# ggerganov/ggml

Measured on NVIDIA H100. Metric: mul_mat_q4_K_4096x11008_n1_weight_throughput, higher is better.
Workload: dtype int8 x int4 (q4_K weights x q8_K activations, dp4a), f32 accumulate

## Files before the change

### ggml_b200/csrc/b200_mm_plan.h

```cpp
#pragma once

#include "b200_internal.h"
#include "b200_quants.cuh"
#include "b200_sb_tasks.cuh"
#include "b200_sb_mma.cuh"

namespace b200 {

struct tma_params {
    const uint8_t * w;
    const float *   x;
    float *         y;
    size_t          nb11;
    int64_t         M, K;
    int32_t         N;
    int32_t         row_bytes;
    int32_t         RB;
    int32_t         P, G;
    int32_t         nchunks;
    int32_t         stage_bytes;
    int32_t         nstages;
    act_layout      L;
};

struct tma_plan {
    tma_params p;
    int grid, block, smem, nc, r;
};

struct sb_params {
    const uint8_t * w; const float * x; float * y;
    int64_t M, K;
    int32_t row_bytes, rows_per_chunk, nchunks, stage_bytes, nstages, ntasks_row;
    unsigned int * counters;
    unsigned int * ctl;
    int32_t ncols; int64_t x_stride;
    int32_t src1_static;
    int32_t src0_static;
    int32_t static_chunks;
    int64_t l2_prefetch_bytes;
    const float * ep_bias; float * ep_y2; float * ep_y3; const float * ep_res;
    unsigned long long * dbg;
    int32_t world, rank;
    int64_t row_offset;
    uint32_t epoch;
    float *    y_peers[8];
    uint32_t * flag_peers[8];
    sb_act A;
};

struct sb_plan { sb_params p; int grid, smem, nw, nc; bool two; };

struct mma_params {
    const uint8_t * w; const float * x; float * y;
    int64_t M, K;
    int32_t row_bytes, ntiles, nslices, ks, ntask_row, pitch, stage_bytes, nstages;
    unsigned int * counters;
    int32_t ncols; int64_t x_stride;
    int32_t src1_static, src0_static;
    int64_t l2_prefetch_bytes;
    const uint8_t * rec_global;
    mma_act A;
};

struct mma_plan { mma_params p; int grid, smem, ng; size_t workspace; };

struct tc2_plan {
    int BN, m_tiles, n_tiles, splitk, chunks, nstages, smem, grid;
    size_t xb_bytes, partial_bytes, scale_bytes, workspace;
};

struct dense_plan { ggml_b200_mul_mat_args b; size_t wbytes; tc2_plan tc; size_t workspace; };

struct mmid_g_plan { int BN, m_tiles, max_tiles, chunks, nstages, smem; size_t xb_bytes, scale_bytes, tab_bytes, perm_bytes, workspace; int64_t n_pairs; };

enum route_kind {
    R_GENERIC,
    R_TMA,
    R_TMA_UNFIT,
    R_SB,
    R_SB_GROUPS,
    R_MMA,
    R_WGMMA,
    R_DENSE,
};

struct mm_plan {
    route_kind kind;
    int64_t group;
    size_t workspace;
    tma_plan tma;
    sb_plan sb, sb_tail;
    mma_plan mma;
    tc2_plan wgmma;
    dense_plan dense;
};

}
```

### ggml_b200/csrc/b200_sb_tasks.cuh

```cuda
#pragma once
#include "b200_quants.cuh"

namespace b200 {

#ifndef B200_HOST_EMU
__device__ __forceinline__ int dp4a_us(uint32_t a, int b, int c) {
    int d;
    asm("dp4a.u32.s32 %0, %1, %2, %3;" : "=r"(d) : "r"(a), "r"(b), "r"(c));
    return d;
}
#else
inline int dp4a_us(uint32_t a, int b, int c) { for (int i = 0; i < 4; ++i) c += (int)((a >> (8 * i)) & 0xFF) * (int)(int8_t)(b >> (8 * i)); return c; }
#endif

template <int T> struct sbfmt;
template <> struct sbfmt<T_Q4_K> { static constexpr int TASK_W = 256, TASK_B = 144, LPR = 16, KQ = 1; };
template <> struct sbfmt<T_Q5_K> { static constexpr int TASK_W = 256, TASK_B = 176, LPR = 16, KQ = 1; };
template <> struct sbfmt<T_Q6_K> { static constexpr int TASK_W = 256, TASK_B = 210, LPR = 16, KQ = 1; };
template <> struct sbfmt<T_Q4_0> { static constexpr int TASK_W = 256, TASK_B = 144, LPR = 16, KQ = 0; };
template <> struct sbfmt<T_Q8_0> { static constexpr int TASK_W = 128, TASK_B = 136, LPR = 32, KQ = 0; };
template <> struct sbfmt<T_Q5_0> { static constexpr int TASK_W = 256, TASK_B = 176, LPR = 16, KQ = 0; };
template <> struct sbfmt<T_IQ4_NL> { static constexpr int TASK_W = 256, TASK_B = 144, LPR = 16, KQ = 0; };
template <> struct sbfmt<T_IQ4_XS> { static constexpr int TASK_W = 256, TASK_B = 136, LPR = 16, KQ = 1; };
template <> struct sbfmt<T_Q4_1> { static constexpr int TASK_W = 256, TASK_B = 160, LPR = 16, KQ = 0; };
// ... 262 lines not shown
        tot -= 32 * off;
#pragma unroll
        for (int j = 0; j < 2; ++j) {
            int p[4] = { 0, 0, 0, 0 };
            const int4 yv0 = lds128(a + (8 * h + j) * 16), yv1 = lds128(a + (8 * h + j + 2) * 16);
            const int4 yv2 = lds128(a + (8 * h + j + 4) * 16), yv3 = lds128(a + (8 * h + j + 6) * 16);
            const int ya[4] = { yv0.x, yv0.y, yv0.z, yv0.w }, yb[4] = { yv1.x, yv1.y, yv1.z, yv1.w };
            const int yc[4] = { yv2.x, yv2.y, yv2.z, yv2.w }, yd4[4] = { yv3.x, yv3.y, yv3.z, yv3.w };
#pragma unroll
            for (int i = 0; i < 4; ++i) {
                const uint32_t la = word(16 * h + 4 * j + i), lb = word(16 * h + 8 + 4 * j + i), qh = word(32 + 8 * h + 4 * j + i);
                p[0] = __dp4a((int)((la & 0x0F0F0F0F)        | ((qh << 4) & 0x30303030)), ya[i], p[0]);
                p[1] = __dp4a((int)((lb & 0x0F0F0F0F)        | ((qh << 2) & 0x30303030)), yb[i], p[1]);
                p[2] = __dp4a((int)(((la >> 4) & 0x0F0F0F0F) | ( qh       & 0x30303030)), yc[i], p[2]);
                p[3] = __dp4a((int)(((lb >> 4) & 0x0F0F0F0F) | ((qh >> 2) & 0x30303030)), yd4[i], p[3]);
            }
            if (j == 0) tot += sbyte<0>(scw0) * p[0] + sbyte<2>(scw0) * p[1] + sbyte<0>(scw1) * p[2] + sbyte<2>(scw1) * p[3];
            else        tot += sbyte<1>(scw0) * p[0] + sbyte<3>(scw0) * p[1] + sbyte<1>(scw1) * p[2] + sbyte<3>(scw1) * p[3];
        }
    }
    const float d = h2f(word(52) & 0xFFFF) * *(const float *)(a + SB_OFF_D);
    return d * (float)tot;
}

template <> __device__ __forceinline__ float task_dot<T_Q5_0>(const uint8_t * w, const uint8_t * rec, int t) {
    const uint8_t * a = rec + (size_t)t * SB_REC;
    uint32_t ww[45];
#pragma unroll
    for (int i = 0; i < 11; ++i) { const int4 v = lds128(w + 16 * i); ww[4 * i] = v.x; ww[4 * i + 1] = v.y; ww[4 * i + 2] = v.z; ww[4 * i + 3] = v.w; }
    ww[44] = 0;
    const int4 sa = lds128(a + SB_OFF_S32), sb = lds128(a + SB_OFF_S32 + 16);
    const int s32[8] = { sa.x, sa.y, sa.z, sa.w, sb.x, sb.y, sb.z, sb.w };
    const int4 da = lds128(a + SB_OFF_D), db = lds128(a + SB_OFF_D + 16);
    const float yd[8] = { __int_as_float(da.x), __int_as_float(da.y), __int_as_float(da.z), __int_as_float(da.w),
                          __int_as_float(db.x), __int_as_float(db.y), __int_as_float(db.z), __int_as_float(db.w) };
    float acc = 0.0f;
#pragma unroll
    for (int b = 0; b < 8; ++b) {
        const int w0 = (22 * b) / 4;
        const bool odd = (b & 1) != 0;
        uint32_t q[4], dbits, qh;
        if (!odd) {
            dbits = ww[w0] & 0xFFFF;
            qh = __funnelshift_r(ww[w0], ww[w0 + 1], 16);
#pragma unroll
            for (int i = 0; i < 4; ++i) q[i] = __funnelshift_r(ww[w0 + 1 + i], ww[w0 + 2 + i], 16);
        } else {
            dbits = ww[w0] >> 16;
            qh = ww[w0 + 1];
#pragma unroll
            for (int i = 0; i < 4; ++i) q[i] = ww[w0 + 2 + i];
        }
        const int4 ylo = lds128(a + (2 * b) * 16), yhi = lds128(a + (2 * b + 1) * 16);
        const int y[8] = { ylo.x, ylo.y, ylo.z, ylo.w, yhi.x, yhi.y, yhi.z, yhi.w };
        const int s = q5_block_dot(q, qh, y) - 16 * s32[b];
        acc += (h2f(dbits) * yd[b]) * (float)s;
    }
    return acc;
}

template <> __device__ __forceinline__ float task_dot<T_IQ4_NL>(const uint8_t * w, const uint8_t * rec, int t) {
    const uint8_t * a = rec + (size_t)t * SB_REC;
    uint32_t ww[37];
#pragma unroll
    for (int i = 0; i < 9; ++i) { const int4 v = lds128(w + 16 * i); ww[4 * i] = v.x; ww[4 * i + 1] = v.y; ww[4 * i + 2] = v.z; ww[4 * i + 3] = v.w; }
    ww[36] = 0;
    const int4 da = lds128(a + SB_OFF_D), db = lds128(a + SB_OFF_D + 16);
    const float yd[8] = { __int_as_float(da.x), __int_as_float(da.y), __int_as_float(da.z), __int_as_float(da.w),
                          __int_as_float(db.x), __int_as_float(db.y), __int_as_float(db.z), __int_as_float(db.w) };
    float acc = 0.0f;
#pragma unroll
    for (int b = 0; b < 8; ++b) {
        const int w0 = (18 * b) / 4;
        const bool odd = (b & 1) != 0;
        uint32_t q[4], dbits;
        if (!odd) {
            dbits = ww[w0] & 0xFFFF;
#pragma unroll
            for (int i = 0; i < 4; ++i) q[i] = __funnelshift_r(ww[w0 + i], ww[w0 + i + 1], 16);
        } else {
            dbits = ww[w0] >> 16;
#pragma unroll
            for (int i = 0; i < 4; ++i) q[i] = ww[w0 + 1 + i];
        }
        const int4 ylo = lds128(a + (2 * b) * 16), yhi = lds128(a + (2 * b + 1) * 16);
        const int yl[4] = { ylo.x, ylo.y, ylo.z, ylo.w }, yh[4] = { yhi.x, yhi.y, yhi.z, yhi.w };
        int s = 0;
#pragma unroll
        for (int i = 0; i < 4; ++i) {
            s = __dp4a((int)iq4nl_lookup4(q[i]), yl[i], s);
            s = __dp4a((int)iq4nl_lookup4(q[i] >> 4), yh[i], s);
        }
        acc += (yd[b] * h2f(dbits)) * (float)s;
    }
    return acc;
}

template <> __device__ __forceinline__ float task_dot<T_IQ4_XS>(const uint8_t * w, const uint8_t * rec, int t) {
    const uint8_t * a = rec + (size_t)t * SB_REC;
    uint32_t ww[34];
#pragma unroll
    for (int i = 0; i < 17; ++i) { const uint2 v = *(const uint2 *)(w + 8 * i); ww[2 * i] = v.x; ww[2 * i + 1] = v.y; }
    int tot = 0;
#pragma unroll
    for (int ib = 0; ib < 8; ++ib) {
        const int4 ylo = lds128(a + (2 * ib) * 16), yhi = lds128(a + (2 * ib + 1) * 16);
        const int yl[4] = { ylo.x, ylo.y, ylo.z, ylo.w }, yh[4] = { yhi.x, yhi.y, yhi.z, yhi.w };
        int s = 0;
#pragma unroll
        for (int i = 0; i < 4; ++i) {
            s = __dp4a((int)iq4nl_lookup4(ww[2 + 4 * ib + i]), yl[i], s);
            s = __dp4a((int)iq4nl_lookup4(ww[2 + 4 * ib + i] >> 4), yh[i], s);
        }
        tot += iq4xs_scale(ww[0], ww[1], ib) * s;
    }
    return (h2f(ww[0] & 0xFFFF) * *(const float *)(a + SB_OFF_D)) * (float)tot;
}

__device__ __forceinline__ void sb_load_q8_1_s(const uint8_t * a, float (&ys)[8]) {
    const int4 sv = lds128(a + SB_OFF_H32);
    const uint32_t u[4] = { (uint32_t)sv.x, (uint32_t)sv.y, (uint32_t)sv.z, (uint32_t)sv.w };
#pragma unroll
    for (int i = 0; i < 4; ++i) { ys[2 * i] = h2f(u[i] & 0xFFFF); ys[2 * i + 1] = h2f(u[i] >> 16); }
}
template <> __device__ __forceinline__ float task_dot<T_Q4_1>(const uint8_t * w, const uint8_t * rec, int t) {
    const uint8_t * a = rec + (size_t)t * SB_REC;
    uint32_t ww[40];
#pragma unroll
    for (int i = 0; i < 10; ++i) { const int4 v = lds128(w + 16 * i); ww[4 * i] = v.x; ww[4 * i + 1] = v.y; ww[4 * i + 2] = v.z; ww[4 * i + 3] = v.w; }
    const int4 da = lds128(a + SB_OFF_D), db = lds128(a + SB_OFF_D + 16);
    const float yd[8] = { __int_as_float(da.x), __int_as_float(da.y), __int_as_float(da.z), __int_as_float(da.w),
                          __int_as_float(db.x), __int_as_float(db.y), __int_as_float(db.z), __int_as_float(db.w) };
    float ys[8];
    sb_load_q8_1_s(a, ys);
    float acc = 0.0f;
#pragma unroll
    for (int b = 0; b < 8; ++b) {
        const int4 ylo = lds128(a + (2 * b) * 16), yhi = lds128(a + (2 * b + 1) * 16);
        const int yl[4] = { ylo.x, ylo.y, ylo.z, ylo.w }, yh[4] = { yhi.x, yhi.y, yhi.z, yhi.w };
        int p0 = 0, p1 = 0;
#pragma unroll
        for (int i = 0; i < 4; ++i) {
            p0 = __dp4a((int)(ww[5 * b + 1 + i] & 0x0F0F0F0F), yl[i], p0);
            p1 = dp4a_us(ww[5 * b + 1 + i] & 0xF0F0F0F0u, yh[i], p1);
        }
        acc += (h2f(ww[5 * b] & 0xFFFF) * yd[b]) * (float)(p0 + (p1 >> 4)) + h2f(ww[5 * b] >> 16) * ys[b];
    }
    return acc;
}
template <> __device__ __forceinline__ float task_dot<T_Q5_1>(const uint8_t * w, const uint8_t * rec, int t) {
    const uint8_t * a = rec + (size_t)t * SB_REC;
    uint32_t ww[48];
#pragma unroll
    for (int i = 0; i < 12; ++i) { const int4 v = lds128(w + 16 * i); ww[4 * i] = v.x; ww[4 * i + 1] = v.y; ww[4 * i + 2] = v.z; ww[4 * i + 3] = v.w; }
    const int4 da = lds128(a + SB_OFF_D), db = lds128(a + SB_OFF_D + 16);
    const float yd[8] = { __int_as_float(da.x), __int_as_float(da.y), __int_as_float(da.z), __int_as_float(da.w),
                          __int_as_float(db.x), __int_as_float(db.y), __int_as_float(db.z), __int_as_float(db.w) };
    float ys[8];
    sb_load_q8_1_s(a, ys);
    float acc = 0.0f;
#pragma unroll
    for (int b = 0; b < 8; ++b) {
        const int4 ylo = lds128(a + (2 * b) * 16), yhi = lds128(a + (2 * b + 1) * 16);
        const int y[8] = { ylo.x, ylo.y, ylo.z, ylo.w, yhi.x, yhi.y, yhi.z, yhi.w };
        const uint32_t q[4] = { ww[6 * b + 2], ww[6 * b + 3], ww[6 * b + 4], ww[6 * b + 5] };
        const int s = q5_block_dot(q, ww[6 * b + 1], y);
        acc += (h2f(ww[6 * b] & 0xFFFF) * yd[b]) * (float)s + h2f(ww[6 * b] >> 16) * ys[b];
    }
    return acc;
}

template <> __device__ __forceinline__ float task_dot<T_Q2_K>(const uint8_t * w, const uint8_t * rec, int t) {
    const uint8_t * a = rec + (size_t)t * SB_REC;
    const uint32_t * wp = (const uint32_t *)w;
    const int4 sa = lds128(a + SB_OFF_S16), sb = lds128(a + SB_OFF_S16 + 16);
    const int s16w[8] = { sa.x, sa.y, sa.z, sa.w, sb.x, sb.y, sb.z, sb.w };
    int isum = 0, msum = 0;
#pragma unroll
    for (int k = 0; k < 4; ++k) {
        const uint32_t scw = wp[k];
        const uint32_t mins = (scw >> 4) & 0x0F0F0F0Fu, scs = scw & 0x0F0F0F0Fu;
        msum = dp2a_lo_su(s16w[2 * k], mins, msum);
        msum = dp2a_hi_su(s16w[2 * k + 1], mins, msum);
#pragma unroll
        for (int gg = 0; gg < 4; ++gg) {
            const int g = 4 * k + gg, h = g >> 3, jj = (g >> 1) & 3, half16 = g & 1;
            const int4 yv = lds128(a + g * 16);
            const int y[4] = { yv.x, yv.y, yv.z, yv.w };
            int p = 0;
#pragma unroll
            for (int i = 0; i < 4; ++i) p = __dp4a((int)((wp[4 + 8 * h + 4 * half16 + i] >> (2 * jj)) & 0x03030303u), y[i], p);
            const int sc = gg == 0 ? ubyte<0>(scs) : gg == 1 ? ubyte<1>(scs) : gg == 2 ? ubyte<2>(scs) : ubyte<3>(scs);
            isum += sc * p;
        }
    }
    const float yd = *(const float *)(a + SB_OFF_D);
    const float dall = yd * h2f(wp[20] & 0xFFFF), dmin = yd * h2f(wp[20] >> 16);
    return dall * (float)isum - dmin * (float)msum;
}

template <> __device__ __forceinline__ float task_dot<T_Q3_K>(const uint8_t * w, const uint8_t * rec, int t) {
    const uint8_t * a = rec + (size_t)t * SB_REC;
    const uint32_t sh = ((uint32_t)(uintptr_t)w & 2) * 8;
    const uint32_t * wa = (const uint32_t *)((uintptr_t)w & ~(uintptr_t)3);
    auto word = [&](int i) { return __funnelshift_r(wa[i], wa[i + 1], sh); };
    const uint32_t s0 = word(24), s1 = word(25), s2 = word(26);
    const uint32_t aux[4] = { ( s0       & 0x0F0F0F0Fu) | (( s2       & 0x03030303u) << 4),
                              ( s1       & 0x0F0F0F0Fu) | (((s2 >> 2) & 0x03030303u) << 4),
                              ((s0 >> 4) & 0x0F0F0F0Fu) | (((s2 >> 4) & 0x03030303u) << 4),
                              ((s1 >> 4) & 0x0F0F0F0Fu) | (((s2 >> 6) & 0x03030303u) << 4) };
    int isum = 0;
#pragma unroll
    for (int g = 0; g < 16; ++g) {
        const int h = g >> 3, jj = (g >> 1) & 3, half16 = g & 1, bit = 4 * h + jj;
        const int4 yv = lds128(a + g * 16);
        const int y[4] = { yv.x, yv.y, yv.z, yv.w };
        int p = 0, low = 0;
#pragma unroll
        for (int i = 0; i < 4; ++i) {
            p   = __dp4a((int)((word(8 + 8 * h + 4 * half16 + i) >> (2 * jj)) & 0x03030303u), y[i], p);
            low = __dp4a((int)(~(word(4 * half16 + i) >> bit) & 0x01010101u), y[i], low);
        }
        const uint32_t ax = aux[g >> 2];
        const int sc = ((g & 3) == 0 ? ubyte<0>(ax) : (g & 3) == 1 ? ubyte<1>(ax) : (g & 3) == 2 ? ubyte<2>(ax) : ubyte<3>(ax)) - 32;
        isum += sc * (p - 4 * low);
    }
    return (h2f(word(27) & 0xFFFF) * *(const float *)(a + SB_OFF_D)) * (float)isum;
}

template <int C, bool FIVE>
__device__ __forceinline__ void q45_chunk2(const uint8_t * qs0, const uint8_t * qs1, const uint32_t (&qh0)[8], const uint32_t (&qh1)[8], const uint8_t * a,
                                            int sa0, int sa1, int sb0, int sb1, int & acc0, int & acc1) {
    const int4 qa0 = lds128(qs0 + 32 * C), qb0 = lds128(qs0 + 32 * C + 16), qa1 = lds128(qs1 + 32 * C), qb1 = lds128(qs1 + 32 * C + 16);
    const uint32_t q0[8] = { (uint32_t)qa0.x, (uint32_t)qa0.y, (uint32_t)qa0.z, (uint32_t)qa0.w, (uint32_t)qb0.x, (uint32_t)qb0.y, (uint32_t)qb0.z, (uint32_t)qb0.w };
    const uint32_t q1[8] = { (uint32_t)qa1.x, (uint32_t)qa1.y, (uint32_t)qa1.z, (uint32_t)qa1.w, (uint32_t)qb1.x, (uint32_t)qb1.y, (uint32_t)qb1.z, (uint32_t)qb1.w };
    int p00 = 0, p01 = 0, p10 = 0, p11 = 0;
#pragma unroll
    for (int h = 0; h < 2; ++h) {
        const int4 ylo = lds128(a + (4 * C + h) * 16), yhi = lds128(a + (4 * C + 2 + h) * 16);
        const int yl[4] = { ylo.x, ylo.y, ylo.z, ylo.w }, yh[4] = { yhi.x, yhi.y, yhi.z, yhi.w };
#pragma unroll
        for (int i = 0; i < 4; ++i) {
            const uint32_t x0 = q0[4 * h + i], x1 = q1[4 * h + i];
            if constexpr (FIVE) {
                const uint32_t h0 = qh0[4 * h + i] >> (2 * C), h1 = qh1[4 * h + i] >> (2 * C);
                p00 = __dp4a((int)((x0 & 0x0F0F0F0F) | ((h0 & 0x01010101) << 4)), yl[i], p00);
                p01 = __dp4a((int)(((x0 >> 4) & 0x0F0F0F0F) | ((h0 & 0x02020202) << 3)), yh[i], p01);
                p10 = __dp4a((int)((x1 & 0x0F0F0F0F) | ((h1 & 0x01010101) << 4)), yl[i], p10);
                p11 = __dp4a((int)(((x1 >> 4) & 0x0F0F0F0F) | ((h1 & 0x02020202) << 3)), yh[i], p11);
            } else {
                p00 = __dp4a((int)(x0 & 0x0F0F0F0F), yl[i], p00);
                p01 = dp4a_us(x0 & 0xF0F0F0F0u, yh[i], p01);
                p10 = __dp4a((int)(x1 & 0x0F0F0F0F), yl[i], p10);
                p11 = dp4a_us(x1 & 0xF0F0F0F0u, yh[i], p11);
            }
        }
    }
    if constexpr (!FIVE) { p01 >>= 4; p11 >>= 4; }
    acc0 += sa0 * p00 + sb0 * p01;
    acc1 += sa1 * p10 + sb1 * p11;
}

template <bool FIVE> __device__ __forceinline__ void q45_task2(const uint8_t * w0, const uint8_t * w1, const uint8_t * rec, int t, float & r0, float & r1) {
    const uint8_t * a = rec + (size_t)t * SB_REC;
    const int4 hdr0 = lds128(w0), hdr1 = lds128(w1);
    const int4 h32 = lds128(a + SB_OFF_H32);
    uint32_t qh0[8] = { 0, 0, 0, 0, 0, 0, 0, 0 }, qh1[8] = { 0, 0, 0, 0, 0, 0, 0, 0 };
    if constexpr (FIVE) {
        const int4 a0 = lds128(w0 + 16), b0 = lds128(w0 + 32), a1 = lds128(w1 + 16), b1 = lds128(w1 + 32);
        qh0[0] = a0.x; qh0[1] = a0.y; qh0[2] = a0.z; qh0[3] = a0.w; qh0[4] = b0.x; qh0[5] = b0.y; qh0[6] = b0.z; qh0[7] = b0.w;
        qh1[0] = a1.x; qh1[1] = a1.y; qh1[2] = a1.z; qh1[3] = a1.w; qh1[4] = b1.x; qh1[5] = b1.y; qh1[6] = b1.z; qh1[7] = b1.w;
    }
    const uint8_t * qs0 = w0 + (FIVE ? 48 : 16), * qs1 = w1 + (FIVE ? 48 : 16);
    int accs[2] = { 0, 0 }, accm[2];
    uint32_t sc_lo[2], sc_hi[2];
#pragma unroll
    for (int r = 0; r < 2; ++r) {
        const int4 & hdr = r == 0 ? hdr0 : hdr1;
        const uint32_t s0 = hdr.y, s1 = hdr.z, s2 = hdr.w;
        const uint32_t mn_lo = s1 & 0x3F3F3F3Fu, mn_hi = ((s2 >> 4) & 0x0F0F0F0Fu) | ((s1 >> 2) & 0x30303030u);
        sc_lo[r] = s0 & 0x3F3F3F3Fu;
        sc_hi[r] = (s2 & 0x0F0F0F0Fu) | ((s0 >> 2) & 0x30303030u);
        int m = dp2a_lo_su(h32.x, mn_lo, 0);
        m = dp2a_hi_su(h32.y, mn_lo, m);
        m = dp2a_lo_su(h32.z, mn_hi, m);
        m = dp2a_hi_su(h32.w, mn_hi, m);
        accm[r] = m;
    }
    q45_chunk2<0, FIVE>(qs0, qs1, qh0, qh1, a, ubyte<0>(sc_lo[0]), ubyte<0>(sc_lo[1]), ubyte<1>(sc_lo[0]), ubyte<1>(sc_lo[1]), accs[0], accs[1]);
    q45_chunk2<1, FIVE>(qs0, qs1, qh0, qh1, a, ubyte<2>(sc_lo[0]), ubyte<2>(sc_lo[1]), ubyte<3>(sc_lo[0]), ubyte<3>(sc_lo[1]), accs[0], accs[1]);
    q45_chunk2<2, FIVE>(qs0, qs1, qh0, qh1, a, ubyte<0>(sc_hi[0]), ubyte<0>(sc_hi[1]), ubyte<1>(sc_hi[0]), ubyte<1>(sc_hi[1]), accs[0], accs[1]);
    q45_chunk2<3, FIVE>(qs0, qs1, qh0, qh1, a, ubyte<2>(sc_hi[0]), ubyte<2>(sc_hi[1]), ubyte<3>(sc_hi[0]), ubyte<3>(sc_hi[1]), accs[0], accs[1]);
    const float yd = *(const float *)(a + SB_OFF_D);
    {
        const float d = h2f((uint32_t)hdr0.x & 0xFFFF) * yd, dmin = h2f((uint32_t)hdr0.x >> 16) * yd;
        r0 = d * (float)accs[0] - dmin * (float)accm[0];
    }
    {
        const float d = h2f((uint32_t)hdr1.x & 0xFFFF) * yd, dmin = h2f((uint32_t)hdr1.x >> 16) * yd;
        r1 = d * (float)accs[1] - dmin * (float)accm[1];
    }
}

template <int C, bool FIVE, int NC>
__device__ __forceinline__ void q45_chunk_nc(const uint8_t * qs, const uint32_t (&qh)[8], const uint8_t * a0, int rec_stride, int ncols, int sc0, int sc1, int (&acc_s)[NC]) {
    const int4 qa = lds128(qs + 32 * C), qb = lds128(qs + 32 * C + 16);
    const uint32_t q[8] = { (uint32_t)qa.x, (uint32_t)qa.y, (uint32_t)qa.z, (uint32_t)qa.w, (uint32_t)qb.x, (uint32_t)qb.y, (uint32_t)qb.z, (uint32_t)qb.w };
    uint32_t lo[8], hi[8];
#pragma unroll
    for (int i = 0; i < 8; ++i) {
        if constexpr (FIVE) {
            const uint32_t hb = qh[i] >> (2 * C);
            lo[i] = (q[i] & 0x0F0F0F0F) | ((hb & 0x01010101) << 4);
            hi[i] = ((q[i] >> 4) & 0x0F0F0F0F) | ((hb & 0x02020202) << 3);
        } else {
            lo[i] = q[i] & 0x0F0F0F0F;
            hi[i] = q[i] & 0xF0F0F0F0u;
        }
    }
#pragma unroll
    for (int c = 0; c < NC; ++c) {
        if (c < ncols) {
            const uint8_t * a = a0 + c * rec_stride;
            int p0 = 0, p1 = 0;
#pragma unroll
            for (int h = 0; h < 2; ++h) {
                const int4 ylo = lds128(a + (4 * C + h) * 16), yhi = lds128(a + (4 * C + 2 + h) * 16);
                const int yl[4] = { ylo.x, ylo.y, ylo.z, ylo.w }, yh[4] = { yhi.x, yhi.y, yhi.z, yhi.w };
#pragma unroll
                for (int i = 0; i < 4; ++i) {
                    p0 = __dp4a((int)lo[4 * h + i], yl[i], p0);
                    if constexpr (FIVE) p1 = __dp4a((int)hi[4 * h + i], yh[i], p1);
                    else                p1 = dp4a_us(hi[4 * h + i], yh[i], p1);
                }
            }
            if constexpr (!FIVE) p1 >>= 4;
            acc_s[c] += sc0 * p0 + sc1 * p1;
        }
    }
}

template <bool FIVE, int NC>
__device__ __forceinline__ void q45_task_nc(const uint8_t * w, const uint8_t * rec, int rec_stride, int t, int ncols, float (&acc)[NC]) {
    const uint8_t * a0 = rec + (size_t)t * SB_REC;
    const int4 hdr = lds128(w);
    uint32_t qh[8] = { 0, 0, 0, 0, 0, 0, 0, 0 };
    if constexpr (FIVE) {
        const int4 ha = lds128(w + 16), hb = lds128(w + 32);
        qh[0] = ha.x; qh[1] = ha.y; qh[2] = ha.z; qh[3] = ha.w; qh[4] = hb.x; qh[5] = hb.y; qh[6] = hb.z; qh[7] = hb.w;
    }
    const uint8_t * qs = w + (FIVE ? 48 : 16);
    const uint32_t s0 = hdr.y, s1 = hdr.z, s2 = hdr.w;
    const uint32_t sc_lo = s0 & 0x3F3F3F3Fu, mn_lo = s1 & 0x3F3F3F3Fu;
    const uint32_t sc_hi = (s2 & 0x0F0F0F0Fu) | ((s0 >> 2) & 0x30303030u);
    const uint32_t mn_hi = ((s2 >> 4) & 0x0F0F0F0Fu) | ((s1 >> 2) & 0x30303030u);
    int acc_s[NC];
#pragma unroll
    for (int c = 0; c < NC; ++c) acc_s[c] = 0;
    q45_chunk_nc<0, FIVE, NC>(qs, qh, a0, rec_stride, ncols, ubyte<0>(sc_lo), ubyte<1>(sc_lo), acc_s);
    q45_chunk_nc<1, FIVE, NC>(qs, qh, a0, rec_stride, ncols, ubyte<2>(sc_lo), ubyte<3>(sc_lo), acc_s);
    q45_chunk_nc<2, FIVE, NC>(qs, qh, a0, rec_stride, ncols, ubyte<0>(sc_hi), ubyte<1>(sc_hi), acc_s);
    q45_chunk_nc<3, FIVE, NC>(qs, qh, a0, rec_stride, ncols, ubyte<2>(sc_hi), ubyte<3>(sc_hi), acc_s);
    const float wd = h2f((uint32_t)hdr.x & 0xFFFF), wm = h2f((uint32_t)hdr.x >> 16);
#pragma unroll
    for (int c = 0; c < NC; ++c) {
        if (c < ncols) {
            const uint8_t * a = a0 + c * rec_stride;
            const int4 h32 = lds128(a + SB_OFF_H32);
            int acc_m = dp2a_lo_su(h32.x, mn_lo, 0);
            acc_m = dp2a_hi_su(h32.y, mn_lo, acc_m);
            acc_m = dp2a_lo_su(h32.z, mn_hi, acc_m);
            acc_m = dp2a_hi_su(h32.w, mn_hi, acc_m);
            const float yd = *(const float *)(a + SB_OFF_D);
            const float d = wd * yd, dmin = wm * yd;
            acc[c] += d * (float)acc_s[c] - dmin * (float)acc_m;
        }
    }
}

template <int T, int NC>
__device__ __forceinline__ void task_dot_nc(const uint8_t * w, const uint8_t * rec, int rec_stride, int t, int ncols, float (&acc)[NC]) {
    if constexpr (T == T_Q4_K)      q45_task_nc<false, NC>(w, rec, rec_stride, t, ncols, acc);
    else if constexpr (T == T_Q5_K) q45_task_nc<true, NC>(w, rec, rec_stride, t, ncols, acc);
    else {
#pragma unroll
        for (int c = 0; c < NC; ++c) if (c < ncols) acc[c] += task_dot<T>(w, rec + c * rec_stride, t);
    }
}

}
```

### ggml_b200/csrc/mmvq_sb.cu

```cuda
#include "b200_internal.h"
#include "b200_mm_plan.h"
#include "b200_quants.cuh"
#include "b200_ptx.cuh"
#include "b200_sb_tasks.cuh"

#include <atomic>
#include <cstdlib>

namespace b200 {

constexpr int SB_MAX_STAGES = 6;

template <int T, int NW, int NC, bool TWO = false>
__global__ void __launch_bounds__((NW + 1) * 32, NC > 1 ? 1 : NW == 8 ? 2 : 4) mmvq_sb_kernel(const sb_params p) {
    using F = sbfmt<T>;
    constexpr int SB_CONSUMER_WARPS = NW;
    constexpr int LPR = F::LPR, RPW = 32 / LPR;
    extern __shared__ __align__(128) uint8_t smem[];
    uint8_t * stages = smem;
    uint8_t * rec    = stages + (size_t)p.nstages * p.stage_bytes;
    uint64_t * full  = (uint64_t *)(rec + NC * p.A.bytes);
    uint64_t * empty = full + SB_MAX_STAGES;
    int * chunk_of   = (int *)(empty + SB_MAX_STAGES);

    const int tid = threadIdx.x, lane = tid & 31, warp = tid >> 5;
    pdl_launch_dependents();
    unsigned long long * dbg = nullptr, * dbg_all = p.dbg;
    if (p.dbg && blockIdx.x == 0) {
        dbg = p.dbg;
        if (tid == 0) dbg[0] = gtime();
    }

    if (tid == 0) {
        for (int s = 0; s < p.nstages; ++s) { mbar_init(&full[s], 1); mbar_init(&empty[s], SB_CONSUMER_WARPS); }
        mbar_fence_init();
    }
    __syncthreads();

    auto issue = [&](int s, int chunk) {
        chunk_of[s] = chunk < p.nchunks ? chunk : -1;
        if (chunk < p.nchunks) {
            const int64_t row0 = (int64_t)chunk * p.rows_per_chunk;
            const int rows = (int)min((int64_t)p.rows_per_chunk, p.M - row0);
            const uint32_t bytes = (uint32_t)rows * (uint32_t)p.row_bytes;
            mbar_expect_tx(&full[s], bytes);
            bulk_g2s(stages + (size_t)s * p.stage_bytes, p.w + (size_t)row0 * p.row_bytes, bytes, &full[s]);
        } else {
            mbar_arrive(&full[s]);
        }
    };

    if (warp == SB_CONSUMER_WARPS) {
        if (lane == 0) {
            if (!p.src0_static) pdl_wait();
            issue(0, (int)blockIdx.x);
            if (p.l2_prefetch_bytes > 0) {
                const int64_t per = ((p.l2_prefetch_bytes + gridDim.x - 1) / gridDim.x + 15) & ~(int64_t)15;
                const int64_t lo = (int64_t)blockIdx.x * per;
                const int64_t hi = min(lo + per, p.l2_prefetch_bytes & ~(int64_t)15);
                for (int64_t o = lo; o < hi; o += 32768) bulk_prefetch_l2(p.w + o, (uint32_t)min((int64_t)32768, hi - o));
            }
            if (dbg) dbg[1] = gtime();
            if (dbg) dbg[2] = gtime();
            int it = 1;
            bool done = (int)blockIdx.x >= p.nchunks;
            if (p.static_chunks) {
                while (!done) {
                    const int s = it % p.nstages;
                    const int chunk = (int)blockIdx.x + it * (int)gridDim.x;
                    if (it >= p.nstages) mbar_wait(&empty[s], (uint32_t)((it / p.nstages) - 1) & 1u);
                    issue(s, chunk);
                    done = chunk >= p.nchunks;
                    ++it;
                }
                return;
            }
            while (!done) {
                const int s = it % p.nstages;
                const int chunk = (int)atomicAdd(&p.counters[0], 1u) + (int)gridDim.x;
                if (it >= p.nstages) mbar_wait(&empty[s], (uint32_t)((it / p.nstages) - 1) & 1u);
                issue(s, chunk);
                done = chunk >= p.nchunks;
                ++it;
            }
            __threadfence();
            if (atomicAdd(&p.counters[1], 1u) == gridDim.x - 1) { p.counters[0] = 0; p.counters[1] = 0; __threadfence(); }
        }
        return;
    }

    if (!p.src1_static) pdl_wait();
    if (dbg && tid == 0) dbg[3] = gtime();
    if (dbg_all && tid == 0) atomicMax(dbg_all + 7, gtime());
    for (int i0 = 2 * warp; i0 < p.ncols * p.A.ntask; i0 += 2 * SB_CONSUMER_WARPS) {
        const int i = i0 + (lane >> 4);
        const bool ok = i < p.ncols * p.A.ntask;
        const int c = NC == 1 ? 0 : (ok ? i / p.A.ntask : 0), t = NC == 1 ? i : (ok ? i % p.A.ntask : 0);
        sb_quantize_task_h<F::KQ != 0, needs_s<T>::value>(p.x + (size_t)c * p.x_stride, ok, rec + c * p.A.bytes, t);
    }
    asm volatile("bar.sync 1, %0;" ::"n"(SB_CONSUMER_WARPS * 32) : "memory");

    const int sub = lane / LPR, l = lane % LPR;
    for (int it = 0;; ++it) {
        const int s = it % p.nstages;
        mbar_wait(&full[s], (uint32_t)(it / p.nstages) & 1u);
        if (dbg && tid == 0 && it == 0) dbg[4] = gtime();
        const int chunk = chunk_of[s];
        if (chunk < 0) { if (dbg && tid == 0) dbg[5] = gtime(); if (dbg_all && tid == 0) atomicMax(dbg_all + 6, gtime()); break; }
        const int64_t row0 = (int64_t)chunk * p.rows_per_chunk;
        const int rows = (int)min((int64_t)p.rows_per_chunk, p.M - row0);
        const uint8_t * st = stages + (size_t)s * p.stage_bytes;
        auto store_row = [&](int64_t grow, float acc) {
            if (p.world == 0) {
                p.y[grow] = acc;
                if (p.ep_bias) {
                    const float v2 = acc + p.ep_bias[grow];
                    p.ep_y2[grow] = v2;
                    if (p.ep_y3) p.ep_y3[grow] = p.ep_res ? v2 + p.ep_res[grow] : gelu_ggml(v2);
                }
            } else {
                const int64_t gi = p.row_offset + grow;
#pragma unroll
                for (int q = 0; q < 8; ++q) if (q < p.world) p.y_peers[q][gi] = acc;
            }
        };
        if constexpr (TWO && NC == 1 && (T == T_Q4_K || T == T_Q5_K)) {
            for (int r0 = warp * RPW * 2; r0 < rows; r0 += SB_CONSUMER_WARPS * RPW * 2) {
                const int r = r0 + 2 * sub;
                float a0 = 0.0f, a1 = 0.0f;
                if (r < rows) {
                    const uint8_t * ra = st + (size_t)r * p.row_bytes, * rb = r + 1 < rows ? ra + p.row_bytes : ra;
                    for (int t = l; t < p.ntasks_row; t += LPR) {
                        float x0, x1;
                        q45_task2<T == T_Q5_K>(ra + (size_t)t * F::TASK_B, rb + (size_t)t * F::TASK_B, rec, t, x0, x1);
                        a0 += x0; a1 += x1;
                    }
                }
#pragma unroll
                for (int o = LPR / 2; o > 0; o >>= 1) { a0 += __shfl_xor_sync(0xffffffffu, a0, o); a1 += __shfl_xor_sync(0xffffffffu, a1, o); }
                if (l == 0 && r < rows) { store_row(row0 + r, a0); if (r + 1 < rows) store_row(row0 + r + 1, a1); }
            }
        } else {
            for (int r0 = warp * RPW; r0 < rows; r0 += SB_CONSUMER_WARPS * RPW) {
                const int r = r0 + sub;
                if constexpr (NC > 1) {
                    float accn[NC];
#pragma unroll
                    for (int c = 0; c < NC; ++c) accn[c] = 0.0f;
                    if (r < rows) {
                        const uint8_t * row = st + (size_t)r * p.row_bytes;
                        for (int t = l; t < p.ntasks_row; t += LPR) task_dot_nc<T, NC>(row + (size_t)t * F::TASK_B, rec, p.A.bytes, t, p.ncols, accn);
                    }
#pragma unroll
                    for (int c = 0; c < NC; ++c) {
#pragma unroll
                        for (int o = LPR / 2; o > 0; o >>= 1) accn[c] += __shfl_xor_sync(0xffffffffu, accn[c], o);
                    }
                    if (l == 0 && r < rows) {
#pragma unroll
                        for (int c = 0; c < NC; ++c) if (c < p.ncols) p.y[(size_t)c * p.M + row0 + r] = accn[c];
                    }
                    continue;
                }
                float acc = 0.0f;
                if (r < rows) {
                    const uint8_t * row = st + (size_t)r * p.row_bytes;
                    for (int t = l; t < p.ntasks_row; t += LPR) acc += task_dot<T>(row + (size_t)t * F::TASK_B, rec, t);
                }
#pragma unroll
                for (int o = LPR / 2; o > 0; o >>= 1) acc += __shfl_xor_sync(0xffffffffu, acc, o);
                if (l == 0 && r < rows) store_row(row0 + r, acc);
            }
        }
        __syncwarp();
        if (lane == 0) mbar_arrive(&empty[s]);
    }
    if (p.src1_static && tid == 0) pdl_wait();
    if (p.world > 0) {
        __threadfence_system();
        asm volatile("bar.sync 1, %0;" ::"n"(SB_CONSUMER_WARPS * 32) : "memory");
        if (tid == 0 && atomicAdd(&p.counters[2], 1u) == gridDim.x - 1) {
            p.counters[2] = 0;
            const uint32_t e = p.epoch ? p.epoch : atomicAdd(&p.ctl[0], 1u) + 1u;
            __threadfence_system();
            for (int q = 0; q < p.world; ++q)
                asm volatile("red.release.sys.global.max.u32 [%0], %1;" ::"l"(p.flag_peers[q] + p.rank), "r"(e) : "memory");
        }
    }
}

__global__ void gather_wait_kernel(const uint32_t * flags, int world, uint32_t epoch, const unsigned int * ctl) {
    const int q = threadIdx.x;
    if (epoch == 0) epoch = ctl[0];
    if (q < world) {
        uint32_t v;
        do {
            asm volatile("ld.acquire.sys.global.u32 %0, [%1];" : "=r"(v) : "l"(flags + q) : "memory");
        } while ((int32_t)(v - epoch) < 0);
    }
    __syncwarp();
    __threadfence_system();
}

static std::atomic<unsigned> g_sb_slot_seq{0};
unsigned int * sb_next_slot(unsigned int * ctl) { return ctl + 64 + (g_sb_slot_seq.fetch_add(1, std::memory_order_relaxed) % 64u) * 8; }

int64_t l2_prefetch_cap() {
    static const int mb = getenv("GGML_B200_SB_L2_MB") ? atoi(getenv("GGML_B200_SB_L2_MB")) : 8;
    return mb > 0 ? (int64_t)mb << 20 : 0;
}

template <int T> static bool make_sb_plan(const ggml_b200_mul_mat_args & a, sb_plan & pl) {
    using F = sbfmt<T>;
    if (a.N < 1 || a.N > 8 || a.ne02 != 1 || a.ne03 != 1 || a.ne12 != 1 || a.ne13 != 1) return false;
    if (a.N > 1 && ((a.nb11 & 3) != 0 || a.nb11 < (size_t)a.K * 4)) return false;
    const int nc = a.N == 1 ? 1 : a.N == 2 ? 2 : a.N <= 4 ? 4 : 8;
    pl.nc = nc;
    if (a.K % 256 != 0 || a.K < 256 || a.M < 1 || a.K > 32768) return false;
    const size_t rb = row_bytes(a.type, a.K);
    if (a.nb01 != rb || ((uintptr_t)a.src0 & 15) != 0 || ((uintptr_t)a.src1 & 3) != 0) return false;
    if ((a.M * rb) % 16 != 0) return false;
    const bool ind = (a.flags & GGML_B200_MM_SRC1_STATIC) != 0 && a.N == 1;
    static const int e_stage_kb = getenv("GGML_B200_SB_STAGE_KB") ? atoi(getenv("GGML_B200_SB_STAGE_KB")) : 0;
    static const int env_stages = getenv("GGML_B200_SB_STAGES")   ? atoi(getenv("GGML_B200_SB_STAGES"))   : 0;
    static const int env_ctas   = getenv("GGML_B200_SB_CTAS")     ? atoi(getenv("GGML_B200_SB_CTAS"))     : 1;
    static const int e_warps    = getenv("GGML_B200_SB_WARPS")    ? atoi(getenv("GGML_B200_SB_WARPS"))    : 0;
    static const int e_resident = getenv("GGML_B200_SB_RESIDENT") ? atoi(getenv("GGML_B200_SB_RESIDENT")) : 0;
    const int env_warps    = e_warps    ? e_warps    : (ind ? 4 : 8);
    const int env_resident = e_resident ? e_resident : (ind ? 4 : 2);
    const int env_stage_kb = e_stage_kb ? e_stage_kb : (ind ? 18 : 36);
    const int SB_CONSUMER_WARPS = (env_warps == 4 && nc == 1) ? 4 : 8;
    pl.nw = SB_CONSUMER_WARPS;
    constexpr int RPW = 32 / F::LPR;
    static const int e_two = getenv("GGML_B200_SB_TWOROW") ? atoi(getenv("GGML_B200_SB_TWOROW")) : 2;
    pl.two = nc == 1 && (T == T_Q4_K || T == T_Q5_K) && (e_two == 1 || (e_two == 2 && !ind && a.K >= 2048 && a.M >= 2048 && (size_t)(SB_CONSUMER_WARPS * RPW * 2) * rb <= 100 * 1024));
    int granule = 1; while ((granule * rb) % 16 != 0) granule *= 2;
    int step = SB_CONSUMER_WARPS * RPW * (pl.two ? 2 : 1); while (step % granule != 0) step *= 2;
    int rpc = (int)(((size_t)env_stage_kb * 1024) / rb) / step * step; if (rpc < step) rpc = step;
    if ((size_t)rpc * rb > 100 * 1024) {
        rpc = granule; while ((size_t)(rpc + granule) * rb <= 48 * 1024) rpc += granule;
        if ((size_t)rpc * rb > 100 * 1024) return false;
    }
    sb_params & p = pl.p;
    p.M = a.M; p.K = a.K;
    p.row_bytes = (int)rb; p.rows_per_chunk = rpc; p.nchunks = (int)((a.M + rpc - 1) / rpc);
    p.stage_bytes = (int)(((size_t)rpc * rb + 127) & ~(size_t)127);
    p.nstages = env_stages;
    p.ntasks_row = (int)(a.K / F::TASK_W);
    p.A = make_sb_act(a.K);
    p.w = nullptr; p.x = nullptr; p.y = nullptr;
    p.ctl = nullptr; p.counters = nullptr; p.dbg = nullptr;
    p.src0_static = (a.flags & GGML_B200_MM_SRC0_STATIC) ? 1 : 0;
    const int64_t l2_cap = l2_prefetch_cap();
    p.l2_prefetch_bytes = (!ind && p.src0_static && l2_cap > 0) ? (int64_t)std::min<size_t>((size_t)a.M * rb, (size_t)l2_cap) : 0;
    p.world = 0; p.rank = 0; p.row_offset = 0; p.epoch = 0;
    p.ep_bias = nullptr; p.ep_y2 = nullptr; p.ep_y3 = nullptr; p.ep_res = nullptr;
    p.src1_static = (a.flags & GGML_B200_MM_SRC1_STATIC) ? 1 : 0;
    static const int e_static = getenv("GGML_B200_SB_STATIC") ? atoi(getenv("GGML_B200_SB_STATIC")) : 0;
    p.static_chunks = (e_static == 1 || (e_static == 2 && !ind)) ? 1 : 0;
    p.ncols = (int32_t)a.N; p.x_stride = a.N > 1 ? (int64_t)(a.nb11 / 4) : 0;
    for (int q = 0; q < 8; ++q) { p.y_peers[q] = nullptr; p.flag_peers[q] = nullptr; }
    auto smem_of = [&]() { return p.nstages * p.stage_bytes + nc * p.A.bytes + 2 * SB_MAX_STAGES * 8 + SB_MAX_STAGES * 4 + 64; };
    const int max_res = nc > 1 ? 1 : SB_CONSUMER_WARPS == 8 ? 2 : 4;
    int ctas = env_ctas < 1 ? 1 : env_ctas > max_res ? max_res : env_ctas;
    int resident = env_resident < ctas ? ctas : env_resident > max_res ? max_res : env_resident;
    if (p.nstages <= 0) {
        p.nstages = 4;
        while (p.nstages > 2 && smem_of() * resident > 226 * 1024) p.nstages--;
    }
    if (p.nstages < 2) p.nstages = 2;
    if (p.nstages > SB_MAX_STAGES) p.nstages = SB_MAX_STAGES;
    while (smem_of() * ctas > 222 * 1024 && p.nstages > 2) p.nstages--;
    while (smem_of() * ctas > 222 * 1024 && ctas > 1) ctas--;
    if (smem_of() > 222 * 1024) return false;
    pl.smem = smem_of();
    pl.grid = sm_count() * ctas;
    if (pl.grid > p.nchunks) pl.grid = p.nchunks;
    return true;
}

static int assign_sb_slot(sb_params & p) {
    p.ctl = control_block();
    if (!p.ctl) return GGML_B200_ECUDA;
    p.counters = sb_next_slot(p.ctl);
    static const bool env_dbg = getenv("GGML_B200_SB_DEBUG") && atoi(getenv("GGML_B200_SB_DEBUG")) != 0;
    static std::atomic<unsigned> dbg_seq{0};
    p.dbg = env_dbg ? (unsigned long long *)(p.ctl + 1024) + (dbg_seq.fetch_add(1, std::memory_order_relaxed) % 32u) * 8 : nullptr;
    return GGML_B200_OK;
}

template <int T, int NW, int NC, bool TWO = false> static int launch_sb_nw(sb_plan & pl, cudaStream_t st) {
    B200_CUDA_TRY(set_max_dynamic_smem<mmvq_sb_kernel<T, NW, NC, TWO>>(222 * 1024));
    B200_CUDA_TRY(launch_pdl(mmvq_sb_kernel<T, NW, NC, TWO>, dim3(pl.grid), dim3((NW + 1) * 32), pl.smem, st, pl.p));
    B200_LAUNCH_CHECK();
    return GGML_B200_OK;
}

template <int T> static int launch_sb_t(const ggml_b200_mul_mat_args & a, sb_plan pl, const ggml_b200_gather * ga, cudaStream_t st, const ggml_b200_epilogue * ep) {
    pl.p.w = (const uint8_t *)a.src0; pl.p.x = a.src1; pl.p.y = a.dst;
    { const int rc = assign_sb_slot(pl.p); if (rc != GGML_B200_OK) return rc; }
    if (ep && ep->bias) {
        pl.p.ep_bias = ep->bias; pl.p.ep_y2 = ep->dst_bias; pl.p.ep_y3 = ep->unary != 0 ? ep->dst_unary : nullptr;
        pl.p.ep_res = ep->unary == 2 ? ep->residual : nullptr;
    }
    if (ga) {
        pl.p.world = ga->world; pl.p.rank = ga->rank; pl.p.row_offset = ga->row_offset; pl.p.epoch = ga->epoch;
        for (int q = 0; q < ga->world; ++q) { pl.p.y_peers[q] = ga->y_peers[q]; pl.p.flag_peers[q] = ga->flag_peers[q]; }
    }
    if (pl.nc > 1 && (ga || (ep && ep->bias))) { set_error("mul_mat: the fused epilogue / gather exist for n = 1 only"); return GGML_B200_EUNSUPPORTED; }
    switch (pl.nc) {
        case 1:
            if constexpr (T == T_Q4_K || T == T_Q5_K) { if (pl.two) return pl.nw == 4 ? launch_sb_nw<T, 4, 1, true>(pl, st) : launch_sb_nw<T, 8, 1, true>(pl, st); }
            return pl.nw == 4 ? launch_sb_nw<T, 4, 1>(pl, st) : launch_sb_nw<T, 8, 1>(pl, st);
        case 2:  return launch_sb_nw<T, 8, 2>(pl, st);
        case 4:  return launch_sb_nw<T, 8, 4>(pl, st);
        default: return launch_sb_nw<T, 8, 8>(pl, st);
    }
}

bool plan_sb(const ggml_b200_mul_mat_args & a, sb_plan & pl) {
    bool ok = false;
    with_format(TC_FORMATS(), a.type, [&](auto t) { ok = make_sb_plan<t>(a, pl); });
    return ok;
}

int launch_sb(const ggml_b200_mul_mat_args & a, const sb_plan & pl, cudaStream_t st, const ggml_b200_gather * ga, const ggml_b200_epilogue * ep) {
    int rc = GGML_B200_EUNSUPPORTED;
    with_format(TC_FORMATS(), a.type, [&](auto t) { rc = launch_sb_t<t>(a, pl, ga, st, ep); });
    return rc;
}

int debug_read_trace(unsigned long long * out) {
    unsigned int * c = control_block();
    if (!c) return GGML_B200_ECUDA;
    B200_CUDA_TRY(cudaDeviceSynchronize());
    B200_CUDA_TRY(cudaMemcpy(out, c + 1024, 32 * 8 * sizeof(unsigned long long), cudaMemcpyDeviceToHost));
    return GGML_B200_OK;
}

int launch_gather_wait(const uint32_t * flags, int world, uint32_t epoch, cudaStream_t st) {
    gather_wait_kernel<<<1, 32, 0, st>>>(flags, world, epoch, control_block());
    B200_LAUNCH_CHECK();
    return GGML_B200_OK;
}

}
```

Before: 2653.

## Hold q4_K/q5_K activations in registers across rows for small-K GEMV

Adds a consumer mode in which each lane loads its slice of the quantized activation record (32 ints plus scales) into registers once, then sweeps weight rows two at a time. Rows are reduced with a butterfly shuffle that packs two rows' partial sums. This removes the repeated shared-memory activation reads per row when K is at most 4096 and there are 4 consumer warps. It costs higher register pressure and possible occupancy loss. The default for static chunk scheduling also changes: it now turns on automatically for independent launches with few chunks per CTA.

```diff
diff --git a/ggml_b200/csrc/b200_mm_plan.h b/ggml_b200/csrc/b200_mm_plan.h
--- a/ggml_b200/csrc/b200_mm_plan.h
+++ b/ggml_b200/csrc/b200_mm_plan.h
@@ -49,7 +49,7 @@
     sb_act A;
 };
 
-struct sb_plan { sb_params p; int grid, smem, nw, nc; bool two; };
+struct sb_plan { sb_params p; int grid, smem, nw, nc; bool two, act_regs; };
 
 struct mma_params {
     const uint8_t * w; const float * x; float * y;
diff --git a/ggml_b200/csrc/b200_sb_tasks.cuh b/ggml_b200/csrc/b200_sb_tasks.cuh
--- a/ggml_b200/csrc/b200_sb_tasks.cuh
+++ b/ggml_b200/csrc/b200_sb_tasks.cuh
@@ -588,6 +588,104 @@
     }
 }
 
+struct q45_acts {
+    int y[32];
+    int h32[2];
+    float d;
+};
+__device__ __forceinline__ void q45_load_acts(const uint8_t * rec, int t, int h, q45_acts & A) {
+    const uint8_t * a = rec + (size_t)t * SB_REC;
+#pragma unroll
+    for (int i = 0; i < 8; ++i) { const int4 v = lds128(a + 128 * h + 16 * i); A.y[4 * i] = v.x; A.y[4 * i + 1] = v.y; A.y[4 * i + 2] = v.z; A.y[4 * i + 3] = v.w; }
+    const uint2 hv = *(const uint2 *)(a + SB_OFF_H32 + 8 * h);
+    A.h32[0] = (int)hv.x; A.h32[1] = (int)hv.y;
+    A.d = *(const float *)(a + SB_OFF_D);
+}
+
+template <int C, bool FIVE>
+__device__ __forceinline__ void q45_chunk_regs(const uint8_t * qs, const uint32_t (&qh)[8], const int (&y)[32], int sc0, int sc1, int & acc_s) {
+    const int4 qa = lds128(qs + 32 * C), qb = lds128(qs + 32 * C + 16);
+    const uint32_t q[8] = { (uint32_t)qa.x, (uint32_t)qa.y, (uint32_t)qa.z, (uint32_t)qa.w, (uint32_t)qb.x, (uint32_t)qb.y, (uint32_t)qb.z, (uint32_t)qb.w };
+    int p0 = 0, p1 = 0;
+#pragma unroll
+    for (int h = 0; h < 2; ++h) {
+#pragma unroll
+        for (int i = 0; i < 4; ++i) {
+            const uint32_t qq = q[4 * h + i];
+            const int yl = y[16 * C + 4 * h + i], yh = y[16 * C + 8 + 4 * h + i];
+            if constexpr (FIVE) {
+                const uint32_t hb = qh[4 * h + i] >> (2 * C);
+                p0 = __dp4a((int)((qq & 0x0F0F0F0F) | ((hb & 0x01010101) << 4)), yl, p0);
+                p1 = __dp4a((int)(((qq >> 4) & 0x0F0F0F0F) | ((hb & 0x02020202) << 3)), yh, p1);
+            } else {
+                p0 = __dp4a((int)(qq & 0x0F0F0F0F), yl, p0);
+                p1 = dp4a_us(qq & 0xF0F0F0F0u, yh, p1);
+            }
+        }
+    }
+    if constexpr (!FIVE) p1 >>= 4;
+    acc_s += sc0 * p0 + sc1 * p1;
+}
+
+template <bool FIVE> __device__ __forceinline__ void q45_half_regs(const uint8_t * w, const q45_acts & A, int h, int & acc_s, int & acc_m, uint32_t & dm) {
+    const int4 hdr = lds128(w);
+    uint32_t qh[8] = { 0, 0, 0, 0, 0, 0, 0, 0 };
+    if constexpr (FIVE) {
+        const int4 ha = lds128(w + 16), hb = lds128(w + 32);
+        const uint32_t raw[8] = { (uint32_t)ha.x, (uint32_t)ha.y, (uint32_t)ha.z, (uint32_t)ha.w, (uint32_t)hb.x, (uint32_t)hb.y, (uint32_t)hb.z, (uint32_t)hb.w };
+#pragma unroll
+        for (int i = 0; i < 8; ++i) qh[i] = raw[i] >> (4 * h);
+    }
+    const uint8_t * qs = w + (FIVE ? 48 : 16) + 64 * h;
+    const uint32_t s0 = hdr.y, s1 = hdr.z, s2 = hdr.w;
+    const uint32_t sc = h ? ((s2 & 0x0F0F0F0Fu) | ((s0 >> 2) & 0x30303030u)) : (s0 & 0x3F3F3F3Fu);
+    const uint32_t mn = h ? (((s2 >> 4) & 0x0F0F0F0Fu) | ((s1 >> 2) & 0x30303030u)) : (s1 & 0x3F3F3F3Fu);
+    acc_m = dp2a_lo_su(A.h32[0], mn, 0);
+    acc_m = dp2a_hi_su(A.h32[1], mn, acc_m);
+    acc_s = 0;
+    q45_chunk_regs<0, FIVE>(qs, qh, A.y, ubyte<0>(sc), ubyte<1>(sc), acc_s);
+    q45_chunk_regs<1, FIVE>(qs, qh, A.y, ubyte<2>(sc), ubyte<3>(sc), acc_s);
+    dm = (uint32_t)hdr.x;
+}
+
+template <bool FIVE, int R> __device__ __forceinline__ float q45_rows_regs(const uint8_t * const (&row)[R], const q45_acts & A, int lane, int ntasks) {
+    const int t = lane >> 1, h = lane & 1;
+    int s[R], m[R];
+    uint32_t dm[R];
+#pragma unroll
+    for (int j = 0; j < R; ++j) { s[j] = 0; m[j] = 0; dm[j] = 0; }
+    if (t < ntasks) {
+#pragma unroll
+        for (int j = 0; j < R; ++j) q45_half_regs<FIVE>(row[j] + (size_t)t * (FIVE ? 176 : 144), A, h, s[j], m[j], dm[j]);
+    }
+    float x[R];
+#pragma unroll
+    for (int j = 0; j < R; ++j) {
+        s[j] += __shfl_xor_sync(0xffffffffu, s[j], 1);
+        m[j] += __shfl_xor_sync(0xffffffffu, m[j], 1);
+        x[j] = 0.0f;
+        if (t < ntasks) {
+            const float d = h2f(dm[j] & 0xFFFF) * A.d, dmin = h2f(dm[j] >> 16) * A.d;
+            x[j] += d * (float)s[j] - dmin * (float)m[j];
+        }
+    }
+#pragma unroll
+    for (int n = R, o = 16; o > 1; o >>= 1) {
+        if (n > 1) {
+            const bool up = (lane & o) != 0;
+#pragma unroll
+            for (int j = 0; j < n / 2; ++j) {
+                const float keep = up ? x[n / 2 + j] : x[j], send = up ? x[j] : x[n / 2 + j];
+                x[j] = keep + __shfl_xor_sync(0xffffffffu, send, o);
+            }
+            n /= 2;
+        } else {
+            x[0] += __shfl_xor_sync(0xffffffffu, x[0], o);
+        }
+    }
+    return x[0];
+}
+
 template <int C, bool FIVE, int NC>
 __device__ __forceinline__ void q45_chunk_nc(const uint8_t * qs, const uint32_t (&qh)[8], const uint8_t * a0, int rec_stride, int ncols, int sc0, int sc1, int (&acc_s)[NC]) {
     const int4 qa = lds128(qs + 32 * C), qb = lds128(qs + 32 * C + 16);
diff --git a/ggml_b200/csrc/mmvq_sb.cu b/ggml_b200/csrc/mmvq_sb.cu
--- a/ggml_b200/csrc/mmvq_sb.cu
+++ b/ggml_b200/csrc/mmvq_sb.cu
@@ -11,7 +11,9 @@
 
 constexpr int SB_MAX_STAGES = 6;
 
-template <int T, int NW, int NC, bool TWO = false>
+enum sb_consume { SB_TASKS = 0, SB_TWO_ROWS = 1, SB_ACT_REGS = 2 };
+
+template <int T, int NW, int NC, int CM = SB_TASKS>
 __global__ void __launch_bounds__((NW + 1) * 32, NC > 1 ? 1 : NW == 8 ? 2 : 4) mmvq_sb_kernel(const sb_params p) {
     using F = sbfmt<T>;
     constexpr int SB_CONSUMER_WARPS = NW;
@@ -99,6 +101,10 @@
         sb_quantize_task_h<F::KQ != 0, needs_s<T>::value>(p.x + (size_t)c * p.x_stride, ok, rec + c * p.A.bytes, t);
     }
     asm volatile("bar.sync 1, %0;" ::"n"(SB_CONSUMER_WARPS * 32) : "memory");
+
+    constexpr int AR = NC == 1 && (T == T_Q4_K || T == T_Q5_K) && CM == SB_ACT_REGS ? 2 : 0;
+    q45_acts acts;
+    if constexpr (AR > 0) { if ((lane >> 1) < p.ntasks_row) q45_load_acts(rec, lane >> 1, lane & 1, acts); }
 
     const int sub = lane / LPR, l = lane % LPR;
     for (int it = 0;; ++it) {
@@ -124,7 +130,16 @@
                 for (int q = 0; q < 8; ++q) if (q < p.world) p.y_peers[q][gi] = acc;
             }
         };
-        if constexpr (TWO && NC == 1 && (T == T_Q4_K || T == T_Q5_K)) {
+        if constexpr (AR > 0) {
+            for (int r0 = warp * AR; r0 < rows; r0 += SB_CONSUMER_WARPS * AR) {
+                const uint8_t * rp[AR];
+#pragma unroll
+                for (int j = 0; j < AR; ++j) rp[j] = st + (size_t)min(r0 + j, rows - 1) * p.row_bytes;
+                const float acc = q45_rows_regs<T == T_Q5_K, AR>(rp, acts, lane, p.ntasks_row);
+                const int r = r0 + lane / (32 / AR);
+                if (lane % (32 / AR) == 0 && r < rows) store_row(row0 + r, acc);
+            }
+        } else if constexpr (CM == SB_TWO_ROWS && NC == 1 && (T == T_Q4_K || T == T_Q5_K)) {
             for (int r0 = warp * RPW * 2; r0 < rows; r0 += SB_CONSUMER_WARPS * RPW * 2) {
                 const int r = r0 + 2 * sub;
                 float a0 = 0.0f, a1 = 0.0f;
@@ -234,6 +249,8 @@
     constexpr int RPW = 32 / F::LPR;
     static const int e_two = getenv("GGML_B200_SB_TWOROW") ? atoi(getenv("GGML_B200_SB_TWOROW")) : 2;
     pl.two = nc == 1 && (T == T_Q4_K || T == T_Q5_K) && (e_two == 1 || (e_two == 2 && !ind && a.K >= 2048 && a.M >= 2048 && (size_t)(SB_CONSUMER_WARPS * RPW * 2) * rb <= 100 * 1024));
+    static const int e_areg = getenv("GGML_B200_SB_ACT_REGS") ? atoi(getenv("GGML_B200_SB_ACT_REGS")) : 1;
+    pl.act_regs = e_areg != 0 && nc == 1 && (T == T_Q4_K || T == T_Q5_K) && a.K <= 16 * 256 && SB_CONSUMER_WARPS == 4;
     int granule = 1; while ((granule * rb) % 16 != 0) granule *= 2;
     int step = SB_CONSUMER_WARPS * RPW * (pl.two ? 2 : 1); while (step % granule != 0) step *= 2;
     int rpc = (int)(((size_t)env_stage_kb * 1024) / rb) / step * step; if (rpc < step) rpc = step;
@@ -256,8 +273,7 @@
     p.world = 0; p.rank = 0; p.row_offset = 0; p.epoch = 0;
     p.ep_bias = nullptr; p.ep_y2 = nullptr; p.ep_y3 = nullptr; p.ep_res = nullptr;
     p.src1_static = (a.flags & GGML_B200_MM_SRC1_STATIC) ? 1 : 0;
-    static const int e_static = getenv("GGML_B200_SB_STATIC") ? atoi(getenv("GGML_B200_SB_STATIC")) : 0;
-    p.static_chunks = (e_static == 1 || (e_static == 2 && !ind)) ? 1 : 0;
+    static const int e_static = getenv("GGML_B200_SB_STATIC") ? atoi(getenv("GGML_B200_SB_STATIC")) : -1;
     p.ncols = (int32_t)a.N; p.x_stride = a.N > 1 ? (int64_t)(a.nb11 / 4) : 0;
     for (int q = 0; q < 8; ++q) { p.y_peers[q] = nullptr; p.flag_peers[q] = nullptr; }
     auto smem_of = [&]() { return p.nstages * p.stage_bytes + nc * p.A.bytes + 2 * SB_MAX_STAGES * 8 + SB_MAX_STAGES * 4 + 64; };
@@ -276,6 +292,7 @@
     pl.smem = smem_of();
     pl.grid = sm_count() * ctas;
     if (pl.grid > p.nchunks) pl.grid = p.nchunks;
+    p.static_chunks = (e_static == 1 || (e_static == 2 && !ind) || (e_static < 0 && ind && p.nchunks <= 16 * pl.grid)) ? 1 : 0;
     return true;
 }
 
@@ -289,9 +306,9 @@
     return GGML_B200_OK;
 }
 
-template <int T, int NW, int NC, bool TWO = false> static int launch_sb_nw(sb_plan & pl, cudaStream_t st) {
-    B200_CUDA_TRY(set_max_dynamic_smem<mmvq_sb_kernel<T, NW, NC, TWO>>(222 * 1024));
-    B200_CUDA_TRY(launch_pdl(mmvq_sb_kernel<T, NW, NC, TWO>, dim3(pl.grid), dim3((NW + 1) * 32), pl.smem, st, pl.p));
+template <int T, int NW, int NC, int CM = SB_TASKS> static int launch_sb_nw(sb_plan & pl, cudaStream_t st) {
+    B200_CUDA_TRY(set_max_dynamic_smem<mmvq_sb_kernel<T, NW, NC, CM>>(222 * 1024));
+    B200_CUDA_TRY(launch_pdl(mmvq_sb_kernel<T, NW, NC, CM>, dim3(pl.grid), dim3((NW + 1) * 32), pl.smem, st, pl.p));
     B200_LAUNCH_CHECK();
     return GGML_B200_OK;
 }
@@ -310,7 +327,10 @@
     if (pl.nc > 1 && (ga || (ep && ep->bias))) { set_error("mul_mat: the fused epilogue / gather exist for n = 1 only"); return GGML_B200_EUNSUPPORTED; }
     switch (pl.nc) {
         case 1:
-            if constexpr (T == T_Q4_K || T == T_Q5_K) { if (pl.two) return pl.nw == 4 ? launch_sb_nw<T, 4, 1, true>(pl, st) : launch_sb_nw<T, 8, 1, true>(pl, st); }
+            if constexpr (T == T_Q4_K || T == T_Q5_K) {
+                if (pl.act_regs) return launch_sb_nw<T, 4, 1, SB_ACT_REGS>(pl, st);
+                if (pl.two) return pl.nw == 4 ? launch_sb_nw<T, 4, 1, SB_TWO_ROWS>(pl, st) : launch_sb_nw<T, 8, 1, SB_TWO_ROWS>(pl, st);
+            }
             return pl.nw == 4 ? launch_sb_nw<T, 4, 1>(pl, st) : launch_sb_nw<T, 8, 1>(pl, st);
         case 2:  return launch_sb_nw<T, 8, 2>(pl, st);
         case 4:  return launch_sb_nw<T, 8, 4>(pl, st);
```

Measured after the change: 2746 (median of 6 runs). 3.5% higher.
